# zsyOAOA/VIRNet

Hardware: AMD Instinct MI355X
Metric: images/sec (256x256x3 denoise fwd) (higher is better)
Workload: dtype f32 (3x3 conv products as split-fp16 MFMA pairs, f32 accumulate)

## Files before the change

include/virnet_hip.h:

```cpp
#ifndef VIRNET_HIP_H
#define VIRNET_HIP_H

#include <stddef.h>
#include <stdint.h>

#ifdef __cplusplus
extern "C" {
#endif

#define VIRNET_ABI_VERSION 5

int virnet_abi_version(void);
const char* virnet_last_error(void);
int virnet_device_count(void);

size_t virnet_packed_weight_floats(int ks, int cin_pad, int n_pad);
int virnet_pack_weight(const float* w, int kind, int cout, int cin, int ks, int cin_pad, int n_pad, int nrep,
                       float* packed, void* stream);

typedef struct virnet_conv_plan {
  int nrep;
  int n_pad;
  int cin_pad;
} virnet_conv_plan;
// ... 15 lines not shown
  float* y_raw;
  float* y_act;
  int n, h, w;
  int cin_pad;
  int cout;
  int n_pad;
  int nrep;
  int ks, stride;
  int epi;
  int nchw_op;
  int crop_h, crop_w;
  int res_sf;
  int in_act;
  float in_slope;
  float slope;
  float mask_slope;
  float clamp_lo, clamp_hi;
} virnet_conv_desc;

int virnet_conv_mfma(const virnet_conv_desc* d, void* stream);
int virnet_conv_mfma_variant(const virnet_conv_desc* d, int out[4]);

size_t virnet_wino_weight_floats(int cin_pad, int n_pad);
int virnet_pack_wino_weight(const float* w_oihw, int dgrad, int cout, int cin, int cin_pad, int n_pad, float* packed, void* stream);
int virnet_conv_wino(const virnet_conv_desc* d, void* stream);

size_t virnet_f16_weight_floats(int cin_pad, int n_pad);
int virnet_pack_f16_weight(const float* w_oihw, int dgrad, int cout, int cin, int cin_pad, int n_pad, float* packed, void* stream);
int virnet_conv_f16(const virnet_conv_desc* d, void* stream);
int virnet_pack_bf16_weight(const float* w_oihw, int dgrad, int cout, int cin, int cin_pad, int n_pad, float* packed, void* stream);
int virnet_conv_bf16(const virnet_conv_desc* d, void* stream);
size_t virnet_f16_convt_weight_floats(int cin, int cout);
int virnet_pack_f16_convt_weight(const float* w_iohw, int cout, int cin, float* packed, void* stream);

size_t virnet_wx4_weight_floats(int cin_pad, int n_pad);
int virnet_pack_wx4_weight(const float* w_oihw, int dgrad, int cout, int cin, int cin_pad, int n_pad, float* packed, void* stream);
int virnet_conv_wx4(const virnet_conv_desc* d, void* stream);
void virnet_conv_wx4_last_plan(int* out4);

enum { VIRNET_LAUNCH_WX4 = 0, VIRNET_LAUNCH_WX4H = 1, VIRNET_LAUNCH_WX4P = 2, VIRNET_LAUNCH_F16 = 3, VIRNET_LAUNCH_S2 = 4, VIRNET_LAUNCH_CONVT = 5 };
typedef struct virnet_conv_launch {
  int form, rows, ng, nrep, variant, slab_base, groups, persistent;
} virnet_conv_launch;
enum { VIRNET_PLAN_WX4 = 0, VIRNET_PLAN_F16 = 1, VIRNET_PLAN_BF16 = 2, VIRNET_PLAN_F16_ENTRY = 3 };
int virnet_conv_plan_query(int family, const virnet_conv_desc* d, int emit_rows, int n_cu,
                           virnet_conv_launch* out, int cap);

size_t virnet_exit_weight_floats(int cin_pad);
int virnet_pack_exit_weight(const float* w_oihw, int cout, int cin, int cin_pad, float* packed, void* stream);
int virnet_conv_exit(const virnet_conv_desc* d, void* stream);

int virnet_set_range_flag(int* device_flag);
int virnet_poison_on_flag(const int* device_flag, float* y, size_t n, void* stream);

typedef struct virnet_thin_desc {
  const float* x;
  const float* wpack;
  const float* bias;
  const float* res;
  float* y;
  int n, h, w, c, cout;
  int crop_h, crop_w;
  int op;
  int res_sf;
  float clamp_lo, clamp_hi;
} virnet_thin_desc;
size_t virnet_thin_weight_floats(int c_pad);
int virnet_pack_thin_weight(const float* w_oihw, int cout, int c, int c_pad, float* packed, void* stream);
int virnet_conv3x3_thin(const virnet_thin_desc* d, void* stream);

typedef struct virnet_pack_desc {
  const float* x;
  const float* vec;
  const float* map;
  float* out;
  int n, c0, h, w, sf;
  int ev;
  int em, mh, mw, msf, map_sqrt;
  int hp, wp;
  int zero_pad;
} virnet_pack_desc;
int virnet_pack_input(const virnet_pack_desc* d, void* stream);
int virnet_conv_f16_entry(const virnet_conv_desc* d, const virnet_pack_desc* e, void* stream);
size_t virnet_entry_weight_floats(int cin, int n_pad);
int virnet_pack_entry_weight(const float* w, int cout, int cin, int n_pad, float* packed, void* stream);
int virnet_conv_entry(const virnet_conv_desc* d, const virnet_pack_desc* e, void* stream);

typedef struct virnet_wgrad_desc {
  const float* x;
  const float* dy;
  const float* in_mul;
  const float* in_add;
  float* dw;
  int* counters;
  int n, h, w, cx, cy;
  int cin, cout;
  int ks, stride;
  int transposed;
  int in_act;
  float in_slope;
} virnet_wgrad_desc;
int virnet_conv_wgrad(const virnet_wgrad_desc* d, void* stream);
size_t virnet_chsplit_bytes(int n, int h, int w, int c);
size_t virnet_conv_wgrad_f16_scratch_bytes(int n, int h, int w, int cx, int cy);
size_t virnet_chsplit_colsum_bytes(int n, int h, int w, int c);
int virnet_chsplit(const float* x, int n, int h, int w, int c, int in_act, float in_slope, const float* in_mul, const float* in_add,
// ... 93 lines not shown
```

virnet_amd/_native.py:

```python
from __future__ import annotations

import ctypes as C
import os
import threading

import torch

_HERE = os.path.dirname(os.path.abspath(__file__))
LIB_PATH = os.environ.get("VIRNET_HIP_LIB") or os.path.join(_HERE, "lib", "libvirnet_hip.so")
ABI_VERSION = 5

c_float_p = C.POINTER(C.c_float)


class ConvPlan(C.Structure):
    _fields_ = [("nrep", C.c_int), ("n_pad", C.c_int), ("cin_pad", C.c_int)]


class ConvDesc(C.Structure):
    _fields_ = [
        ("x", C.c_void_p), ("wpack", C.c_void_p), ("bias", C.c_void_p), ("res", C.c_void_p),
        ("mul", C.c_void_p), ("add", C.c_void_p), ("mask", C.c_void_p), ("in_mul", C.c_void_p), ("in_add", C.c_void_p),
        ("y_raw", C.c_void_p), ("y_act", C.c_void_p),
        ("n", C.c_int), ("h", C.c_int), ("w", C.c_int), ("cin_pad", C.c_int), ("cout", C.c_int),
# ... 13 lines not shown

class PackDesc(C.Structure):
    _fields_ = [
        ("x", C.c_void_p), ("vec", C.c_void_p), ("map", C.c_void_p), ("out", C.c_void_p),
        ("n", C.c_int), ("c0", C.c_int), ("h", C.c_int), ("w", C.c_int), ("sf", C.c_int),
        ("ev", C.c_int),
        ("em", C.c_int), ("mh", C.c_int), ("mw", C.c_int), ("msf", C.c_int), ("map_sqrt", C.c_int),
        ("hp", C.c_int), ("wp", C.c_int), ("zero_pad", C.c_int),
    ]


class ImageGradDesc(C.Structure):
    _fields_ = [
        ("dres", C.c_void_p), ("ga", C.c_void_p), ("wa", C.c_void_p), ("gb", C.c_void_p), ("wb", C.c_void_p), ("dx", C.c_void_p),
        ("n", C.c_int), ("c0", C.c_int), ("h", C.c_int), ("w", C.c_int), ("sf", C.c_int),
        ("hp", C.c_int), ("wp", C.c_int), ("ca", C.c_int), ("cina", C.c_int),
        ("cb", C.c_int), ("cinb", C.c_int), ("accumulate", C.c_int),
    ]


class ThinDesc(C.Structure):
    _fields_ = [
        ("x", C.c_void_p), ("wpack", C.c_void_p), ("bias", C.c_void_p), ("res", C.c_void_p), ("y", C.c_void_p),
        ("n", C.c_int), ("h", C.c_int), ("w", C.c_int), ("c", C.c_int), ("cout", C.c_int),
        ("crop_h", C.c_int), ("crop_w", C.c_int), ("op", C.c_int), ("res_sf", C.c_int),
        ("clamp_lo", C.c_float), ("clamp_hi", C.c_float),
    ]


class WgradDesc(C.Structure):
    _fields_ = [
        ("x", C.c_void_p), ("dy", C.c_void_p), ("in_mul", C.c_void_p), ("in_add", C.c_void_p), ("dw", C.c_void_p),
        ("counters", C.c_void_p), ("n", C.c_int), ("h", C.c_int), ("w", C.c_int), ("cx", C.c_int), ("cy", C.c_int),
        ("cin", C.c_int), ("cout", C.c_int), ("ks", C.c_int), ("stride", C.c_int), ("transposed", C.c_int),
        ("in_act", C.c_int), ("in_slope", C.c_float),
    ]


class KnetLayer(C.Structure):
    _fields_ = [(k, C.c_void_p) for k in ("w1pack", "b1", "w2pack", "b2", "caw1", "cab1", "caw2", "cab2")]


class SftWeights(C.Structure):
    _fields_ = [
        ("w1", C.c_void_p), ("b1", C.c_void_p), ("w2", C.c_void_p), ("b2", C.c_void_p),
        ("wm", C.c_void_p), ("bm", C.c_void_p), ("wa", C.c_void_p), ("ba", C.c_void_p),
        ("e", C.c_int), ("nf1", C.c_int), ("nf2", C.c_int), ("nf", C.c_int),
    ]


EPI_NHWC, EPI_CONVT, EPI_NCHW = 0, 1, 2
GAP_MEAN, GAP_EXPCLAMP, GAP_KINFO = 0, 1, 2
NCHW_PLAIN, NCHW_ADD, NCHW_EXPCLAMP = 0, 1, 2
PLAN_WX4, PLAN_F16, PLAN_BF16, PLAN_F16_ENTRY = 0, 1, 2, 3

SYMBOLS = [
    ("virnet_abi_version", C.c_int, []),
    ("virnet_last_error", C.c_char_p, []),
    ("virnet_device_count", C.c_int, []),
    ("virnet_packed_weight_floats", C.c_size_t, [C.c_int, C.c_int, C.c_int]),
    ("virnet_pack_weight", C.c_int, [C.c_void_p, C.c_int, C.c_int, C.c_int, C.c_int, C.c_int, C.c_int, C.c_int,
                                     C.c_void_p, C.c_void_p]),
    ("virnet_conv_get_plan", C.c_int, [C.c_int, C.c_int, C.c_int, C.c_int, C.POINTER(ConvPlan)]),
    ("virnet_conv_mfma", C.c_int, [C.POINTER(ConvDesc), C.c_void_p]),
    ("virnet_conv_mfma_variant", C.c_int, [C.POINTER(ConvDesc), C.POINTER(C.c_int * 4)]),
    ("virnet_wino_weight_floats", C.c_size_t, [C.c_int, C.c_int]),
    ("virnet_pack_wino_weight", C.c_int, [C.c_void_p, C.c_int, C.c_int, C.c_int, C.c_int, C.c_int, C.c_void_p, C.c_void_p]),
    ("virnet_conv_wino", C.c_int, [C.POINTER(ConvDesc), C.c_void_p]),
    ("virnet_f16_weight_floats", C.c_size_t, [C.c_int, C.c_int]),
    ("virnet_pack_f16_weight", C.c_int, [C.c_void_p, C.c_int, C.c_int, C.c_int, C.c_int, C.c_int, C.c_void_p, C.c_void_p]),
    ("virnet_conv_f16", C.c_int, [C.POINTER(ConvDesc), C.c_void_p]),
    ("virnet_wx4_weight_floats", C.c_size_t, [C.c_int, C.c_int]),
    ("virnet_pack_wx4_weight", C.c_int, [C.c_void_p, C.c_int, C.c_int, C.c_int, C.c_int, C.c_int, C.c_void_p, C.c_void_p]),
    ("virnet_conv_wx4", C.c_int, [C.POINTER(ConvDesc), C.c_void_p]),
    ("virnet_conv_wx4_last_plan", None, [C.POINTER(C.c_int)]),
    ("virnet_conv_plan_query", C.c_int, [C.c_int, C.POINTER(ConvDesc), C.c_int, C.c_int, C.POINTER(ConvLaunch), C.c_int]),
    ("virnet_exit_weight_floats", C.c_size_t, [C.c_int]),
    ("virnet_pack_exit_weight", C.c_int, [C.c_void_p, C.c_int, C.c_int, C.c_int, C.c_void_p, C.c_void_p]),
    ("virnet_conv_exit", C.c_int, [C.POINTER(ConvDesc), C.c_void_p]),
    ("virnet_set_range_flag", C.c_int, [C.c_void_p]),
    ("virnet_poison_on_flag", C.c_int, [C.c_void_p, C.c_void_p, C.c_size_t, C.c_void_p]),
    ("virnet_pack_bf16_weight", C.c_int, [C.c_void_p, C.c_int, C.c_int, C.c_int, C.c_int, C.c_int, C.c_void_p, C.c_void_p]),
    ("virnet_conv_bf16", C.c_int, [C.POINTER(ConvDesc), C.c_void_p]),
    ("virnet_f16_convt_weight_floats", C.c_size_t, [C.c_int, C.c_int]),
    ("virnet_pack_f16_convt_weight", C.c_int, [C.c_void_p, C.c_int, C.c_int, C.c_void_p, C.c_void_p]),
    ("virnet_pack_input", C.c_int, [C.POINTER(PackDesc), C.c_void_p]),
    ("virnet_conv_f16_entry", C.c_int, [C.POINTER(ConvDesc), C.POINTER(PackDesc), C.c_void_p]),
    ("virnet_entry_weight_floats", C.c_size_t, [C.c_int, C.c_int]),
    ("virnet_pack_entry_weight", C.c_int, [C.c_void_p, C.c_int, C.c_int, C.c_int, C.c_void_p, C.c_void_p]),
    ("virnet_conv_entry", C.c_int, [C.POINTER(ConvDesc), C.POINTER(PackDesc), C.c_void_p]),
    ("virnet_thin_weight_floats", C.c_size_t, [C.c_int]),
    ("virnet_pack_thin_weight", C.c_int, [C.c_void_p, C.c_int, C.c_int, C.c_int, C.c_void_p, C.c_void_p]),
    ("virnet_conv3x3_thin", C.c_int, [C.POINTER(ThinDesc), C.c_void_p]),
    ("virnet_conv_wgrad", C.c_int, [C.POINTER(WgradDesc), C.c_void_p]),
    ("virnet_sft_backward", C.c_int, [C.c_void_p, C.c_void_p, C.c_void_p, C.c_void_p, C.c_void_p, C.c_float, C.c_void_p, C.c_void_p, C.c_void_p,
                                      C.c_int, C.c_long, C.c_int, C.c_void_p]),
    ("virnet_chsplit_bytes", C.c_size_t, [C.c_int, C.c_int, C.c_int, C.c_int]),
    ("virnet_conv_wgrad_f16_scratch_bytes", C.c_size_t, [C.c_int, C.c_int, C.c_int, C.c_int, C.c_int]),
    ("virnet_chsplit_colsum_bytes", C.c_size_t, [C.c_int, C.c_int, C.c_int, C.c_int]),
    ("virnet_chsplit", C.c_int, [C.c_void_p, C.c_int, C.c_int, C.c_int, C.c_int, C.c_int, C.c_float, C.c_void_p, C.c_void_p, C.c_int,
                                 C.c_void_p, C.c_void_p, C.c_void_p, C.c_int, C.c_void_p]),
    ("virnet_conv_wgrad_f16", C.c_int, [C.c_void_p, C.c_void_p, C.c_void_p, C.c_void_p, C.c_int, C.c_int, C.c_int, C.c_int, C.c_int, C.c_int, C.c_int,
                                        C.c_int, C.c_void_p]),
    ("virnet_chsplit_s2_bytes", C.c_size_t, [C.c_int, C.c_int, C.c_int, C.c_int]),
    ("virnet_chsplit_s2_colsum_bytes", C.c_size_t, [C.c_int, C.c_int, C.c_int, C.c_int]),
    ("virnet_chsplit_s2", C.c_int, [C.c_void_p, C.c_int, C.c_int, C.c_int, C.c_int, C.c_int, C.c_float, C.c_void_p, C.c_void_p, C.c_int,
                                    C.c_void_p, C.c_void_p, C.c_void_p, C.c_int, C.c_void_p]),
    ("virnet_conv_wgrad_f16_s2_scratch_bytes", C.c_size_t, [C.c_int, C.c_int, C.c_int, C.c_int, C.c_int]),
    ("virnet_conv_wgrad_f16_s2", C.c_int, [C.c_void_p, C.c_void_p, C.c_void_p, C.c_void_p, C.c_int, C.c_int, C.c_int, C.c_int, C.c_int, C.c_int,
                                           C.c_int, C.c_int, C.c_int, C.c_void_p]),
    ("virnet_conv_emit_ok", C.c_int, [C.POINTER(ConvDesc), C.c_int, C.POINTER(C.c_int)]),
    ("virnet_conv_f16_emit", C.c_int, [C.POINTER(ConvDesc), C.POINTER(TEmit), C.c_int, C.c_void_p]),
    ("virnet_conv_wx4_emit", C.c_int, [C.POINTER(ConvDesc), C.POINTER(TEmit), C.c_void_p]),
    ("virnet_colpart_reduce", C.c_int, [C.c_void_p, C.c_void_p, C.c_long, C.c_int, C.c_int, C.c_void_p]),
    ("virnet_conv_wgrad_f16_db", C.c_int, [C.c_void_p, C.c_void_p, C.c_void_p, C.c_void_p, C.c_int, C.c_int, C.c_int, C.c_int, C.c_int, C.c_int, C.c_int,
                                           C.c_int, C.c_void_p, C.c_void_p, C.c_long, C.c_int, C.c_void_p]),
    ("virnet_colsum", C.c_int, [C.c_void_p, C.c_void_p, C.c_long, C.c_int, C.c_int, C.c_void_p]),
    ("virnet_zero_stuff2", C.c_int, [C.c_void_p, C.c_void_p, C.c_int, C.c_int, C.c_int, C.c_int, C.c_void_p]),
    ("virnet_space_to_depth2", C.c_int, [C.c_void_p, C.c_void_p, C.c_int, C.c_int, C.c_int, C.c_int, C.c_void_p]),
    ("virnet_pack_input_backward", C.c_int, [C.c_void_p, C.c_int, C.c_int, C.c_void_p, C.c_void_p, C.c_int, C.c_int, C.c_int, C.c_int,
                                             C.c_int, C.c_int, C.c_int, C.c_void_p]),
    ("virnet_image_grad", C.c_int, [C.POINTER(ImageGradDesc), C.c_void_p]),
    ("virnet_conv_head_s4", C.c_int, [C.c_void_p, C.c_void_p, C.c_void_p, C.c_int, C.c_int, C.c_int, C.c_int, C.c_int,
                                      C.c_void_p]),
    ("virnet_conv_head_s4_wgrad", C.c_int, [C.c_void_p, C.c_void_p, C.c_void_p, C.c_int, C.c_int, C.c_int, C.c_int, C.c_int,
                                            C.c_void_p]),
    ("virnet_conv_head_s4_dgrad", C.c_int, [C.c_void_p, C.c_void_p, C.c_void_p, C.c_int, C.c_int, C.c_int, C.c_int, C.c_int,
                                            C.c_void_p]),
    ("virnet_gap_nchw", C.c_int, [C.c_void_p, C.c_void_p, C.c_int, C.c_int, C.c_int, C.c_int, C.c_int, C.c_float,
                                  C.c_float, C.c_void_p]),
    ("virnet_ca_gate", C.c_int, [C.c_void_p, C.c_void_p, C.c_void_p, C.c_void_p, C.c_void_p, C.c_void_p, C.c_int, C.c_int,
                                 C.c_int, C.c_int, C.c_int, C.c_void_p]),
    ("virnet_knet_body", C.c_int, [C.c_void_p, C.c_void_p, C.c_void_p, C.c_int, C.c_int, C.c_int, C.c_int, C.c_int, C.c_int, C.c_void_p]),
    ("virnet_scale_add", C.c_int, [C.c_void_p, C.c_void_p, C.c_void_p, C.c_void_p, C.c_int, C.c_int, C.c_int, C.c_void_p]),
# ... 60 lines not shown
```

virnet_amd/csrc/api.cpp:

```cpp
#include "common.h"
#include <cstdlib>
namespace virnet { int* range_flag_ptr(); int store_nt_for(size_t bytes); }
#include "../../include/virnet_hip.h"

namespace virnet {

char* error_slot() {
  static thread_local char buf[512] = {0};
  return buf;
}

int set_error(const char* fmt, ...) {
  va_list ap;
  va_start(ap, fmt);
  vsnprintf(error_slot(), 512, fmt, ap);
  va_end(ap);
  return 1;
}

static thread_local int* g_range_flag[64] = {nullptr};

int* range_flag_ptr() {
  int dev = 0;
  if (hipGetDevice(&dev) != hipSuccess || dev < 0 || dev > 63) return nullptr;
  return g_range_flag[dev];
}

int store_nt_for(size_t bytes) {
  const char* e = getenv("VIRNET_NT_STORE_MB");
  const long limit = e ? atol(e) : 128;
  return limit > 0 && bytes > (size_t)limit * 1048576u;
}

}

extern "C" int virnet_abi_version(void) { return VIRNET_ABI_VERSION; }

extern "C" const char* virnet_last_error(void) { return virnet::error_slot(); }

extern "C" int virnet_device_count(void) {
  int n = 0;
  hipError_t e = hipGetDeviceCount(&n);
  if (e != hipSuccess) {
    virnet::set_error("hipGetDeviceCount: %s", hipGetErrorString(e));
    return -1;
  }
  return n;
}

extern "C" int virnet_set_range_flag(int* device_flag) {
  int dev = 0;
  hipError_t e = hipGetDevice(&dev);
  if (e != hipSuccess) return virnet::set_error("virnet_set_range_flag: hipGetDevice: %s", hipGetErrorString(e));
  if (dev < 0 || dev > 63) return virnet::set_error("virnet_set_range_flag: device %d out of range", dev);
  virnet::g_range_flag[dev] = device_flag;
  return 0;
}
```

virnet_amd/engine.py:

```python
from __future__ import annotations

from typing import List, Optional, Tuple

import torch

from . import _native as nat
from . import ops

Tensor = torch.Tensor

LOG_MAX = 4.605170185988092
LOG_MIN = -23.025850929940457
K_LOG_MIN = -9.210340371976182


def _prep(x: Tensor, chn: int, name: str = "x") -> Tensor:
    if x.dim() != 4:
        raise ValueError(f"{name} must be [N,C,H,W], got {tuple(x.shape)}")
    if x.shape[1] != chn:
        raise ValueError(f"{name} has {x.shape[1]} channels, the network was built for {chn}")
    if not x.is_cuda:
        raise RuntimeError(f"{name} is on {x.device}: the VIRNet HIP path runs on a ROCm device only (no CPU fallback)")
    if x.dtype != torch.float32:
        raise TypeError(f"{name} must be float32 (the reference is fp32 end to end), got {x.dtype}")
# ... 90 lines not shown
        if ev + em != rnet.extra_chn:
            raise ValueError(f"conditioning has {ev + em} channels, the network was built for {rnet.extra_chn}")
        if extra_map is not None:
            extra_map = _prep(extra_map, em, "extra maps")
        if extra_vec is not None:
            extra_vec = extra_vec.detach().contiguous()
    feed_head = mode in ("input", "both")
    feed_down = mode in ("down", "both")
    cond = None
    rec = None
    if feed_down:
        if extra_map is None:
            cond = _Cond(extra_vec, None, 0, ev)
        else:
            rec = ops.pack_input(x_in, Hp, Wp, sf=sf, vec=extra_vec if feed_head else None,
                                 map_=extra_map if feed_head else None, map_sf=map_sf, map_sqrt=map_sqrt)
            crec = rec if feed_head else ops.pack_input(x_in, Hp, Wp, sf=sf, vec=extra_vec, map_=extra_map,
                                                        map_sf=map_sf, map_sqrt=map_sqrt)
            cond = _Cond(None, crec, rnet.in_chn, ev + em)
    if rec is not None:
        x, _ = ops.conv_mfma(rec, rnet.head.packed(), want_raw=True)
    else:
        x = ops.conv_entry(x_in, rnet.head.packed(), Hp, Wp, sf=sf, vec=extra_vec if feed_head else None,
                           map_=extra_map if feed_head else None, map_sf=map_sf, map_sqrt=map_sqrt)
    if cond is not None and cond.vec is not None and ops._env("VIRNET_SFT_MULTI", "1") != "0":
        atts = [a for lvl in rnet.down_path for blk in lvl.body if blk.extra_chn > 0 for a in (blk.sft1, blk.sft2)]
        if atts:
            cond.pre = {id(a): ma for a, ma in zip(atts, ops.sft_vec_multi(cond.vec, atts))}
    bridges: List[Tensor] = []
    for ii, lvl in enumerate(rnet.down_path):
        for blk in lvl.body:
            x = _res_block(x, blk, cond, ii)
        if ii + 1 < len(rnet.down_path):
            bridges.append(x)
            x, _ = ops.conv_mfma(x, lvl.downsampler.packed(), stride=2, want_raw=True)
    for jj, up in enumerate(rnet.up_path):
        x, _ = ops.conv_mfma(x, up.upsampler.packed(), res=bridges[-jj - 1], want_raw=True)
        for blk in up.body:
            x = _res_block(x, blk, None, 0)
    return _conv_planar(x, rnet.tail, (H, W), op=nat.NCHW_ADD, res=x_in, res_sf=sf)


FP32_FORM = "wino"


class RangeOverflowRepaired(RuntimeWarning):
    """A forward of the deferred guard mode left fp16's range: its outputs were NaN on the device until the repair that this warning
    announces (the same input repeated with the fp32 kernels, written into the same output tensors)."""


_GUARD_WARNING = ("VIRNet HIP path: an activation left fp16's range in a split-fp16 convolution (|x| >= 65504, or >= ~6.5e3 in the "
                  "Winograd form); the forward was repeated with the fp32 kernels")
MAX_PENDING = 2


def guard_check_mode() -> str:
    mode = ops._env("VIRNET_GUARD_CHECK", "sync")
    if mode not in ("sync", "deferred"):
        raise ValueError(f"VIRNET_GUARD_CHECK={mode!r}: expected sync or deferred")
    return mode


def _pending_list() -> list:
    lst = getattr(nat.tls, "guard_pending", None)
    if lst is None:
        lst = nat.tls.guard_pending = []
    return lst


def _settle(block: bool, keep: int = 0) -> None:
    import warnings
    pend = _pending_list()
    while pend:
        pinned, ev, run, outs, dev, stream = pend[0]
        if not ev.query():
            if not block or len(pend) <= keep:
                return
            ev.synchronize()
        pend.pop(0)
        overflowed = bool(int(pinned[0]))
        _pinned_pool().append(pinned)
        if overflowed:
            _GUARD_STATS["reruns"] += 1
            with torch.no_grad(), torch.cuda.device(dev), torch.cuda.stream(stream), ops.forward_scope(form=FP32_FORM):
                res = run()
                for o, r in zip(outs, res if isinstance(res, tuple) else (res,)):
                    o.copy_(r)
            warnings.warn(_GUARD_WARNING + " (deferred check: its outputs were NaN until now)", RangeOverflowRepaired, stacklevel=4)


def _pinned_pool() -> list:
    pool = getattr(nat.tls, "guard_pinned", None)
    if pool is None:
        pool = nat.tls.guard_pinned = []
    return pool


def guard_poll(block: bool = True) -> None:
    _settle(block)


def _range_guarded(run, x: Tensor):
    import warnings
    guarded = ops._f16_family() and ops.range_guard_enabled() and not torch.cuda.is_current_stream_capturing()
    deferred = guarded and guard_check_mode() == "deferred"
    if guarded:
        _settle(block=False)
        flag = ops.range_flag(x.device)
        flag.zero_()
    with ops.forward_scope():
        out = run()
    if deferred:
        outs = out if isinstance(out, tuple) else (out,)
        for o in outs:
            ops.poison_on_flag(flag, o)
        pool = _pinned_pool()
        if pool:
            pinned = pool.pop()
        else:
            with nat.capture_lock:
                pinned = torch.zeros(1, dtype=torch.int32).pin_memory()
        pinned.copy_(flag, non_blocking=True)
        ev = torch.cuda.Event()
        ev.record()
        _pending_list().append((pinned, ev, run, outs, x.device, torch.cuda.current_stream()))
        _settle(block=True, keep=MAX_PENDING)
    elif guarded and ops.range_overflowed(x.device):
        warnings.warn(_GUARD_WARNING, RuntimeWarning, stacklevel=3)
        _GUARD_STATS["reruns"] += 1
        with ops.forward_scope(form=FP32_FORM):
            out = run()
    if guarded:
        _GUARD_STATS["forwards"] += 1
    return out


_GUARD_STATS = {"forwards": 0, "reruns": 0}


def guard_stats(reset: bool = False) -> dict:
    out = dict(_GUARD_STATS)
    if reset:
        _GUARD_STATS["forwards"] = _GUARD_STATS["reruns"] = 0
    return out


def denoise_forward(net, x: Tensor) -> Tuple[Tensor, Tensor]:
    x = _prep(x, net.SNet.in_channels)
    with torch.cuda.device(x.device):
        return _range_guarded(lambda: _denoise_forward(net, x), x)


def _denoise_forward(net, x: Tensor) -> Tuple[Tensor, Tensor]:
    sigma = snet_forward(net.SNet, x, mode="sigma")
    if net.noise_cond:
        if net.SNet.noise_avg:
            raise RuntimeError("VIRAttResUNet(noise_avg=True, noise_cond=True): the [N,C,1,1] variance cannot be "
                               "padded or concatenated with the image (same failure as the reference)")
        mu = rnet_forward(net.RNet, x, extra_map=sigma, map_sqrt=True)
    else:
        mu = rnet_forward(net.RNet, x)
    return mu, sigma


def sisr_forward(net, x: Tensor, sf) -> Tuple[Tensor, Tensor, Tensor]:
    x = _prep(x, net.SNet.in_channels)
    with torch.cuda.device(x.device):
        return _range_guarded(lambda: _sisr_forward(net, x, sf), x)


def _sisr_forward(net, x: Tensor, sf) -> Tuple[Tensor, Tensor, Tensor]:
    if int(sf) != sf or sf < 1:
        raise ValueError(f"sf must be a positive integer, got {sf}")
    sf = int(sf)
    n = x.shape[0]
    sigma = snet_forward(net.SNet, x, mode="sigma")
    kinfo = knet_forward(net.KNet, x)
    vec_parts, emap = [], None
    if net.kernel_cond:
        vec_parts.append(kinfo.view(n, -1))
# ... 9 lines not shown
```

virnet_amd/graph.py:

```python
from __future__ import annotations

import operator
import os
import threading
import warnings
import weakref
from collections import OrderedDict
from typing import Callable, Iterable, Optional, Tuple

import torch

from . import _native as nat
from . import ops


_EPOCH = [0]
FULL_CHECK_EVERY = 64
_VERSIONS = operator.attrgetter("_version")


def _bump(*_a, **_k):
    _EPOCH[0] += 1


def bump_epoch() -> None:
    _EPOCH[0] += 1


_HOOKS = []


def _install_hooks() -> None:
    if not _HOOKS:
        _HOOKS.append(torch.nn.modules.module.register_module_parameter_registration_hook(_bump))
        _HOOKS.append(torch.nn.modules.module.register_module_module_registration_hook(_bump))


_CAPTURE_LOCK = nat.capture_lock


def _env_stamp() -> int:
    data = getattr(os.environ, "_data", None)
    return hash(tuple(data.items())) if data is not None else hash(tuple(sorted(os.environ.items())))


_GRAVEYARD: list = []


def _release(holder=None) -> None:
    with _CAPTURE_LOCK:
        if holder is not None:
            holder.clear()
        del _GRAVEYARD[:]


class RangeOverflow(RuntimeError):
    """Raised by a ``check="deferred"`` GraphedForward when the PREVIOUS replay staged an operand outside fp16's range."""


class GraphedForward:

    def __init__(self, fn: Callable, warmup: int = 2, params: Optional[Callable[[], Iterable[torch.Tensor]]] = None,
                 check: str = "sync", auto_after: int = 0, fresh: bool = False, max_graphs: int = 0):
        if check not in ("sync", "deferred", "off"):
            raise ValueError(f"check={check!r}: expected 'sync', 'deferred' or 'off'")
        _install_hooks()
        self.fn, self.warmup, self.check = fn, warmup, check
        self.auto_after, self.fresh, self.max_graphs = auto_after, fresh, max_graphs
        self._params = params
        self._stamp = None
        self._plist = None
        self._calls = 0
        self._graphs: "OrderedDict[Tuple, Tuple]" = OrderedDict()
        self._seen: dict = {}
        self._pending = None
        self.reruns = 0
        self.replays = 0

    def _walk(self):
        plist = list(self._params())
        return (_EPOCH[0], plist, tuple((id(p), p.data_ptr()) for p in plist))

    def _fingerprint(self):
        if self._params is None:
            return None
        self._calls += 1
        if self._plist is None or self._plist[0] != _EPOCH[0] or self._calls % FULL_CHECK_EVERY == 0:
            self._plist = self._walk()
        return (self._plist[2], tuple(map(_VERSIONS, self._plist[1])))

    def _guard_flag(self, device) -> Optional[torch.Tensor]:
        if self.check == "off" or not (ops._f16_family() and ops.range_guard_enabled()):
            return None
        return ops.range_flag(device)

    def _capture(self, x: torch.Tensor, args: tuple):
        static_x = x.clone()
        flag = self._guard_flag(x.device)
        side = torch.cuda.Stream()
        side.wait_stream(torch.cuda.current_stream())
        with torch.cuda.stream(side), torch.no_grad():
            for _ in range(self.warmup):
                self.fn(static_x, *args)
        torch.cuda.current_stream().wait_stream(side)
        with _CAPTURE_LOCK:
            _sweep_registry()
            _release()
            pinned = torch.zeros(1, dtype=torch.int32).pin_memory() if flag is not None else None
            graph = torch.cuda.CUDAGraph()
            with torch.no_grad(), torch.cuda.graph(graph, capture_error_mode="thread_local"):
                if flag is not None:
                    flag.zero_()
                out = self.fn(static_x, *args)
                out = out if isinstance(out, tuple) else (out,)
                if flag is not None:
                    for o in out:
                        ops.poison_on_flag(flag, o)
                    if pinned is not None and self.check == "sync":
                        pinned.copy_(flag, non_blocking=True)
        return graph, static_x, out, flag, pinned

    def poll(self) -> None:
        if self._pending is None:
            return
        pinned, ev = self._pending
        self._pending = None
        ev.synchronize()
        if int(pinned.item()):
            raise RangeOverflow("the previous graph replay staged an operand outside fp16's range: its outputs are NaN-filled; "
                                "run that input through the eager forward (which repeats it with the fp32 kernels)")

    def __call__(self, x: torch.Tensor, *args):
        if self.check == "deferred":
            self.poll()
        stamp = self._fingerprint()
        if stamp != self._stamp:
            _release(self._graphs)
            self._seen.clear()
            self._stamp = stamp
        key = (tuple(x.shape), x.device.index, args, _env_stamp())
        hit = self._graphs.get(key)
        if hit is None:
            if self.auto_after > 0:
                seen = self._seen.get(key, 0)
                if seen < self.auto_after:
                    if len(self._seen) > 4096:
                        self._seen.clear()
                    self._seen[key] = seen + 1
                    return self.fn(x, *args)
            with torch.cuda.device(x.device):
                hit = self._graphs[key] = self._capture(x, args)
            self._seen.pop(key, None)
            while self.max_graphs > 0 and len(self._graphs) > self.max_graphs:
                with _CAPTURE_LOCK:
                    self._graphs.popitem(last=False)
        elif self.max_graphs > 0:
            self._graphs.move_to_end(key)
        graph, static_x, out, flag, pinned = hit
        static_x.copy_(x)
        graph.replay()
        self.replays += 1
        done = None
        if flag is not None and self.check == "sync":
            done = torch.cuda.Event()
            done.record()
        if self.fresh:
            ret = tuple(torch.empty_like(o) for o in out)
            torch._foreach_copy_(list(ret), list(out))
        else:
            ret = out
        if flag is not None:
            if self.check == "deferred":
                pinned.copy_(flag, non_blocking=True)
                ev = torch.cuda.Event()
                ev.record()
                self._pending = (pinned, ev)
                return ret if len(ret) > 1 else ret[0]
            done.synchronize()
            if int(pinned[0]):
                warnings.warn("VIRNet HIP path: an activation left fp16's range in a replayed graph; this input was repeated eagerly "
                              "with the fp32 kernels", RuntimeWarning, stacklevel=2)
                self.reruns += 1
                from . import engine
                with torch.no_grad(), torch.cuda.device(x.device), ops.forward_scope(form=engine.FP32_FORM):
                    res = self.fn(static_x, *args)
                for o, r in zip(ret, res if isinstance(res, tuple) else (res,)):
                    o.copy_(r)
        return ret if len(ret) > 1 else ret[0]

    def reset(self) -> None:
        _release(self._graphs)
        self._seen.clear()
        self._pending = None

    def __del__(self):
        try:
            _GRAVEYARD.extend(self._graphs.values())
        except Exception:
            pass


AUTO_AFTER = 2


class no_autograph:

    def __enter__(self):
        nat.tls.autograph_off = getattr(nat.tls, "autograph_off", 0) + 1
        return self

    def __exit__(self, *exc):
        nat.tls.autograph_off -= 1
        return False


_REGISTRY: list = []
_REGISTRY_LOCK = threading.Lock()


def _sweep_registry() -> None:
    with _REGISTRY_LOCK:
        dead = [e for e in _REGISTRY if e[0]() is None or not e[1].is_alive()]
        for e in dead:
            _REGISTRY.remove(e)
    for _, _, gf in dead:
        gf.reset()


def _auto_state(module, fn) -> GraphedForward:
    per_thread = getattr(nat.tls, "autograph", None)
    if per_thread is None:
        per_thread = nat.tls.autograph = weakref.WeakKeyDictionary()
# ... 26 lines not shown
```

virnet_amd/ops.py:

```python
from __future__ import annotations

import ctypes as C
import os
from dataclasses import dataclass
from typing import Optional, Tuple

import torch

from . import _native as nat

Tensor = torch.Tensor


@dataclass
class PackedWeight:
    w: Tensor
    bias: Optional[Tensor]
    ks: int
    cout: int
    cin_real: int
    cin_pad: int
    n_pad: int
    nrep: int
    transposed: bool
# ... 133 lines not shown
    if cout < min_cout:
        return False
    th, tw = (h + 15) // 16, (w + 31) // 32
    fill = (h * w) / float(th * 16 * tw * 32)
    if th * tw < min_tiles or fill < min_fill:
        return False
    if deterministic:
        return True
    if n * th * tw * ((cout + 95) // 96) >= min_wgs:
        return True
    return cout % 96 == 0 and n * ((h + 7) // 8) * tw * (cout // 32) >= min_slab_wgs


def pack_wx4_weight(weight: Tensor, *, dgrad: bool = False) -> Tensor:
    lib = nat.load()
    weight = weight.detach()
    _dev_check(weight, "weight")
    cout, cin, kh, kw = weight.shape
    if (kh, kw) != (3, 3):
        raise ValueError("the Winograd form is for 3x3 kernels")
    rows, ks = (cin, cout) if dgrad else (cout, cin)
    if rows % 32:
        raise ValueError(f"virnet_conv_wx4 stores multiples of 32 channels, got {rows}")
    cin_pad = (ks + 15) // 16 * 16
    out = torch.empty(lib.virnet_wx4_weight_floats(cin_pad, rows), dtype=torch.float32, device=weight.device)
    nat.check(lib.virnet_pack_wx4_weight(nat.ptr(weight), int(dgrad), cout, cin, cin_pad, rows, nat.ptr(out), nat.stream_handle()),
              "pack_wx4_weight")
    return out


def wx4_last_plan() -> dict:
    out = (C.c_int * 4)()
    nat.load().virnet_conv_wx4_last_plan(out)
    return {"rows": out[0], "persistent": bool(out[1]), "slabs": out[2], "launches": out[3]}


def conv_plan_query(family: int, desc: "nat.ConvDesc", *, emit_rows: int = 0, n_cu: int = 0) -> list:
    lib = nat.load()
    out = (nat.ConvLaunch * 4)()
    n = lib.virnet_conv_plan_query(family, C.byref(desc), emit_rows, n_cu, out, 4)
    if n < 0:
        nat.check(n, "conv_plan_query")
    return [{k: getattr(out[i], k) for k, _ in nat.ConvLaunch._fields_} for i in range(n)]


def _wino_enabled() -> bool:
    return conv_form() == "wino"


def range_guard_enabled() -> bool:
    return _env("VIRNET_RANGE_GUARD", "1") != "0"


def range_flag(device: torch.device) -> Optional[Tensor]:
    if not range_guard_enabled():
        return None
    idx = device.index if device.index is not None else torch.cuda.current_device()
    flags = getattr(nat.tls, "range_flags", None)
    if flags is None:
        flags = nat.tls.range_flags = {}
    flag = flags.get(idx)
    if flag is None:
        flag = torch.zeros(1, dtype=torch.int32, device=torch.device("cuda", idx))
        with torch.cuda.device(idx):
            nat.check(nat.load().virnet_set_range_flag(nat.ptr(flag)), "set_range_flag")
        flags[idx] = flag
    return flag


def range_overflowed(device: torch.device, *, reset: bool = True) -> bool:
    flag = range_flag(device)
    if flag is None or not bool(flag.item()):
        return False
    if reset:
        flag.zero_()
    return True


def poison_on_flag(flag: Tensor, y: Tensor) -> None:
    nat.check(nat.load().virnet_poison_on_flag(nat.ptr(flag), nat.ptr(y), y.numel(), nat.stream_handle()), "poison_on_flag")


def pack_f16_weight(weight: Tensor, *, dgrad: bool = False, bf16: bool = False) -> Tensor:
    lib = nat.load()
    weight = weight.detach()
    _dev_check(weight, "weight")
    cout, cin, kh, kw = weight.shape
    if (kh, kw) != (3, 3):
        raise ValueError("the split-fp16 form is for 3x3 kernels")
    rows, ks = (cin, cout) if dgrad else (cout, cin)
    n_pad = (rows + 31) // 32 * 32
    cin_pad = (ks + 15) // 16 * 16
    out = torch.empty(lib.virnet_f16_weight_floats(cin_pad, n_pad), dtype=torch.float32, device=weight.device)
    fn = lib.virnet_pack_bf16_weight if bf16 else lib.virnet_pack_f16_weight
    nat.check(fn(nat.ptr(weight), int(dgrad), cout, cin, cin_pad, n_pad, nat.ptr(out), nat.stream_handle()), "pack_f16_weight")
    return out


def pack_wino_weight(weight: Tensor, *, dgrad: bool = False) -> Tensor:
    lib = nat.load()
    weight = weight.detach()
    _dev_check(weight, "weight")
    cout, cin, kh, kw = weight.shape
    if (kh, kw) != (3, 3):
        raise ValueError("the Winograd form is for 3x3 kernels")
    rows, ks = (cin, cout) if dgrad else (cout, cin)
    if rows % 32:
        raise ValueError(f"the Winograd kernel stores multiples of 32 channels, got {rows}")
    cin_pad = (ks + 15) // 16 * 16
    out = torch.empty(lib.virnet_wino_weight_floats(cin_pad, rows), dtype=torch.float32, device=weight.device)
    nat.check(lib.virnet_pack_wino_weight(nat.ptr(weight), int(dgrad), cout, cin, cin_pad, rows, nat.ptr(out), nat.stream_handle()),
              "pack_wino_weight")
    return out


def _dev_check(t: Tensor, name: str) -> None:
    if not t.is_cuda:
        raise RuntimeError(f"{name} is on {t.device}: the VIRNet HIP path needs tensors on a ROCm device "
                           f"(no CPU fallback exists; move the module and inputs with .cuda())")
    if t.dtype != torch.float32:
        raise TypeError(f"{name} must be float32, got {t.dtype}")
    if not t.is_contiguous():
        raise ValueError(f"{name} must be contiguous")


def get_plan(ks: int, stride: int, cin: int, gemm_n: int) -> nat.ConvPlan:
    plan = nat.ConvPlan()
    nat.check(nat.load().virnet_conv_get_plan(ks, stride, cin, gemm_n, C.byref(plan)), "conv_get_plan")
    return plan


def pack_weight(weight: Tensor, bias: Optional[Tensor], *, transposed: bool = False, stride: int = 1,
                dgrad: bool = False) -> PackedWeight:
# ... 875 lines not shown
```

Before: 1590.

## Replace device range flag with mapped pinned host flag slots

The fp16 range-guard flag now lives in host-mapped coherent pinned memory with per-thread slots, so kernels write it directly into host-visible memory. The per-forward device zero_, the pinned copy and the .item() readback are replaced with a host-side store when the stream is idle and a spin on hipStreamQuery followed by an atomic host load. Deferred mode and graphs get dedicated slots with reusable events. This cuts per-forward launches and synchronisation cost, in exchange for kernels doing flag writes over the host-coherent path and added slot-management complexity.

```diff
diff --git a/include/virnet_hip.h b/include/virnet_hip.h
--- a/include/virnet_hip.h
+++ b/include/virnet_hip.h
@@ -91,6 +91,15 @@
 
 int virnet_set_range_flag(int* device_flag);
 int virnet_poison_on_flag(const int* device_flag, float* y, size_t n, void* stream);
+
+#define VIRNET_RANGE_SLOTS 16
+#define VIRNET_RANGE_STRIDE 64
+int virnet_range_select(int slot);
+int* virnet_range_flag_ptr(int slot, int host_side);
+int virnet_range_begin(int slot, void* stream);
+int virnet_range_end(void* stream, int* overflowed);
+int virnet_range_record(void* stream, void** ticket);
+int virnet_range_query(void* ticket, int wait, int* landed, int* overflowed);
 
 typedef struct virnet_thin_desc {
   const float* x;
diff --git a/virnet_amd/_native.py b/virnet_amd/_native.py
--- a/virnet_amd/_native.py
+++ b/virnet_amd/_native.py
@@ -89,6 +89,7 @@
 EPI_NHWC, EPI_CONVT, EPI_NCHW = 0, 1, 2
 GAP_MEAN, GAP_EXPCLAMP, GAP_KINFO = 0, 1, 2
 NCHW_PLAIN, NCHW_ADD, NCHW_EXPCLAMP = 0, 1, 2
+RANGE_SLOTS = 16
 PLAN_WX4, PLAN_F16, PLAN_BF16, PLAN_F16_ENTRY = 0, 1, 2, 3
 
 SYMBOLS = [
@@ -117,6 +118,12 @@
     ("virnet_conv_exit", C.c_int, [C.POINTER(ConvDesc), C.c_void_p]),
     ("virnet_set_range_flag", C.c_int, [C.c_void_p]),
     ("virnet_poison_on_flag", C.c_int, [C.c_void_p, C.c_void_p, C.c_size_t, C.c_void_p]),
+    ("virnet_range_select", C.c_int, [C.c_int]),
+    ("virnet_range_flag_ptr", C.c_void_p, [C.c_int, C.c_int]),
+    ("virnet_range_begin", C.c_int, [C.c_int, C.c_void_p]),
+    ("virnet_range_end", C.c_int, [C.c_void_p, C.POINTER(C.c_int)]),
+    ("virnet_range_record", C.c_int, [C.c_void_p, C.POINTER(C.c_void_p)]),
+    ("virnet_range_query", C.c_int, [C.c_void_p, C.c_int, C.POINTER(C.c_int), C.POINTER(C.c_int)]),
     ("virnet_pack_bf16_weight", C.c_int, [C.c_void_p, C.c_int, C.c_int, C.c_int, C.c_int, C.c_int, C.c_void_p, C.c_void_p]),
     ("virnet_conv_bf16", C.c_int, [C.POINTER(ConvDesc), C.c_void_p]),
     ("virnet_f16_convt_weight_floats", C.c_size_t, [C.c_int, C.c_int]),
diff --git a/virnet_amd/csrc/api.cpp b/virnet_amd/csrc/api.cpp
--- a/virnet_amd/csrc/api.cpp
+++ b/virnet_amd/csrc/api.cpp
@@ -1,5 +1,7 @@
 #include "common.h"
 #include <cstdlib>
+#include <cstring>
+#include <mutex>
 namespace virnet { int* range_flag_ptr(); int store_nt_for(size_t bytes); }
 #include "../../include/virnet_hip.h"
 
@@ -18,12 +20,83 @@
   return 1;
 }
 
-static thread_local int* g_range_flag[64] = {nullptr};
+struct RangeSlot {
+  int* host;
+  int* dev;
+  hipEvent_t ev;
+};
+
+struct RangeBlock {
+  RangeSlot slot[VIRNET_RANGE_SLOTS];
+  RangeBlock* next;
+};
+
+static std::mutex g_range_mutex;
+static RangeBlock* g_range_free[64] = {nullptr};
+
+struct RangeThread {
+  RangeBlock* block[64] = {nullptr};
+  int cur[64] = {0};
+  int* user[64] = {nullptr};
+  bool idle[64] = {false};
+  void* idle_stream[64] = {nullptr};
+  ~RangeThread() {
+    std::lock_guard<std::mutex> lock(g_range_mutex);
+    for (int d = 0; d < 64; ++d)
+      if (block[d]) {
+        block[d]->next = g_range_free[d];
+        g_range_free[d] = block[d];
+      }
+  }
+};
+static thread_local RangeThread g_range;
+
+static int current_device(const char* who, int* dev) {
+  hipError_t e = hipGetDevice(dev);
+  if (e != hipSuccess) return set_error("%s: hipGetDevice: %s", who, hipGetErrorString(e));
+  if (*dev < 0 || *dev > 63) return set_error("%s: device %d out of range", who, *dev);
+  return 0;
+}
+
+static RangeBlock* range_block(int dev) {
+  RangeThread& t = g_range;
+  if (t.block[dev]) return t.block[dev];
+  RangeBlock* b = nullptr;
+  {
+    std::lock_guard<std::mutex> lock(g_range_mutex);
+    b = g_range_free[dev];
+    if (b) g_range_free[dev] = b->next;
+  }
+  if (!b) {
+    void* host = nullptr;
+    void* devp = nullptr;
+    hipError_t e = hipHostMalloc(&host, (size_t)VIRNET_RANGE_SLOTS * VIRNET_RANGE_STRIDE, hipHostMallocMapped | hipHostMallocCoherent);
+    if (e == hipSuccess) e = hipHostGetDevicePointer(&devp, host, 0);
+    if (e != hipSuccess) {
+      set_error("range flag: hipHostMalloc: %s", hipGetErrorString(e));
+      return nullptr;
+    }
+    memset(host, 0, (size_t)VIRNET_RANGE_SLOTS * VIRNET_RANGE_STRIDE);
+    b = new RangeBlock();
+    for (int i = 0; i < VIRNET_RANGE_SLOTS; ++i) {
+      b->slot[i].host = reinterpret_cast<int*>(static_cast<char*>(host) + (size_t)i * VIRNET_RANGE_STRIDE);
+      b->slot[i].dev = reinterpret_cast<int*>(static_cast<char*>(devp) + (size_t)i * VIRNET_RANGE_STRIDE);
+      b->slot[i].ev = nullptr;
+    }
+  }
+  b->next = nullptr;
+  t.block[dev] = b;
+  t.idle[dev] = false;
+  return b;
+}
 
 int* range_flag_ptr() {
   int dev = 0;
   if (hipGetDevice(&dev) != hipSuccess || dev < 0 || dev > 63) return nullptr;
-  return g_range_flag[dev];
+  RangeThread& t = g_range;
+  t.idle[dev] = false;
+  if (t.user[dev]) return t.user[dev];
+  return t.block[dev] ? t.block[dev]->slot[t.cur[dev]].dev : nullptr;
 }
 
 int store_nt_for(size_t bytes) {
@@ -50,9 +123,110 @@
 
 extern "C" int virnet_set_range_flag(int* device_flag) {
   int dev = 0;
-  hipError_t e = hipGetDevice(&dev);
-  if (e != hipSuccess) return virnet::set_error("virnet_set_range_flag: hipGetDevice: %s", hipGetErrorString(e));
-  if (dev < 0 || dev > 63) return virnet::set_error("virnet_set_range_flag: device %d out of range", dev);
-  virnet::g_range_flag[dev] = device_flag;
-  return 0;
-}
+  if (virnet::current_device("virnet_set_range_flag", &dev)) return 1;
+  virnet::g_range.user[dev] = device_flag;
+  virnet::g_range.idle[dev] = false;
+  return 0;
+}
+
+extern "C" int virnet_range_select(int slot) {
+  int dev = 0;
+  if (virnet::current_device("virnet_range_select", &dev)) return 1;
+  VIRNET_REQUIRE(slot >= 0 && slot < VIRNET_RANGE_SLOTS, "virnet_range_select: slot %d out of range", slot);
+  if (!virnet::range_block(dev)) return 1;
+  virnet::g_range.cur[dev] = slot;
+  return 0;
+}
+
+extern "C" int* virnet_range_flag_ptr(int slot, int host_side) {
+  int dev = 0;
+  if (virnet::current_device("virnet_range_flag_ptr", &dev)) return nullptr;
+  if (slot < 0 || slot >= VIRNET_RANGE_SLOTS) {
+    virnet::set_error("virnet_range_flag_ptr: slot %d out of range", slot);
+    return nullptr;
+  }
+  virnet::RangeBlock* b = virnet::range_block(dev);
+  if (!b) return nullptr;
+  return host_side ? b->slot[slot].host : b->slot[slot].dev;
+}
+
+extern "C" int virnet_range_begin(int slot, void* stream) {
+  int dev = 0;
+  if (virnet::current_device("virnet_range_begin", &dev)) return 1;
+  virnet::RangeThread& t = virnet::g_range;
+  hipStream_t s = static_cast<hipStream_t>(stream);
+  if (t.user[dev]) {
+    hipError_t e = hipMemsetAsync(t.user[dev], 0, sizeof(int), s);
+    VIRNET_REQUIRE(e == hipSuccess, "virnet_range_begin: hipMemsetAsync: %s", hipGetErrorString(e));
+    return 0;
+  }
+  if (virnet_range_select(slot)) return 1;
+  const virnet::RangeSlot& w = t.block[dev]->slot[slot];
+  bool host_store = t.idle[dev] && t.idle_stream[dev] == stream;
+  if (host_store) {
+    hipStreamCaptureStatus st = hipStreamCaptureStatusNone;
+    host_store = hipStreamIsCapturing(s, &st) == hipSuccess && st == hipStreamCaptureStatusNone;
+  }
+  if (host_store) {
+    __atomic_store_n(w.host, 0, __ATOMIC_RELEASE);
+  } else {
+    hipError_t e = hipMemsetAsync(w.dev, 0, sizeof(int), s);
+    VIRNET_REQUIRE(e == hipSuccess, "virnet_range_begin: hipMemsetAsync: %s", hipGetErrorString(e));
+  }
+  t.idle[dev] = false;
+  return 0;
+}
+
+extern "C" int virnet_range_end(void* stream, int* overflowed) {
+  int dev = 0;
+  if (virnet::current_device("virnet_range_end", &dev)) return 1;
+  VIRNET_REQUIRE(overflowed != nullptr, "virnet_range_end: NULL pointer");
+  virnet::RangeThread& t = virnet::g_range;
+  VIRNET_REQUIRE(t.user[dev] || t.block[dev], "virnet_range_end: no range flag on device %d in this thread", dev);
+  hipError_t e;
+  while ((e = hipStreamQuery(static_cast<hipStream_t>(stream))) == hipErrorNotReady) __builtin_ia32_pause();
+  VIRNET_REQUIRE(e == hipSuccess, "virnet_range_end: hipStreamQuery: %s", hipGetErrorString(e));
+  if (t.user[dev]) {
+    int v = 0;
+    e = hipMemcpy(&v, t.user[dev], sizeof(int), hipMemcpyDeviceToHost);
+    VIRNET_REQUIRE(e == hipSuccess, "virnet_range_end: hipMemcpy: %s", hipGetErrorString(e));
+    *overflowed = v != 0;
+    return 0;
+  }
+  *overflowed = __atomic_load_n(t.block[dev]->slot[t.cur[dev]].host, __ATOMIC_ACQUIRE) != 0;
+  t.idle[dev] = true;
+  t.idle_stream[dev] = stream;
+  return 0;
+}
+
+extern "C" int virnet_range_record(void* stream, void** ticket) {
+  int dev = 0;
+  if (virnet::current_device("virnet_range_record", &dev)) return 1;
+  VIRNET_REQUIRE(ticket != nullptr, "virnet_range_record: NULL pointer");
+  virnet::RangeThread& t = virnet::g_range;
+  VIRNET_REQUIRE(t.block[dev] && !t.user[dev], "virnet_range_record: the thread's current flag on device %d is not the library's", dev);
+  virnet::RangeSlot& w = t.block[dev]->slot[t.cur[dev]];
+  hipError_t e = hipSuccess;
+  if (!w.ev) e = hipEventCreateWithFlags(&w.ev, hipEventDisableTiming);
+  if (e == hipSuccess) e = hipEventRecord(w.ev, static_cast<hipStream_t>(stream));
+  VIRNET_REQUIRE(e == hipSuccess, "virnet_range_record: %s", hipGetErrorString(e));
+  *ticket = &w;
+  return 0;
+}
+
+extern "C" int virnet_range_query(void* ticket, int wait, int* landed, int* overflowed) {
+  VIRNET_REQUIRE(ticket && landed && overflowed, "virnet_range_query: NULL pointer");
+  virnet::RangeSlot* w = static_cast<virnet::RangeSlot*>(ticket);
+  VIRNET_REQUIRE(w->ev != nullptr, "virnet_range_query: not a recorded ticket");
+  hipError_t e = hipEventQuery(w->ev);
+  if (e == hipErrorNotReady && wait) e = hipEventSynchronize(w->ev);
+  if (e == hipErrorNotReady) {
+    *landed = 0;
+    *overflowed = 0;
+    return 0;
+  }
+  VIRNET_REQUIRE(e == hipSuccess, "virnet_range_query: %s", hipGetErrorString(e));
+  *landed = 1;
+  *overflowed = __atomic_load_n(w->host, __ATOMIC_ACQUIRE) != 0;
+  return 0;
+}
diff --git a/virnet_amd/engine.py b/virnet_amd/engine.py
--- a/virnet_amd/engine.py
+++ b/virnet_amd/engine.py
@@ -166,6 +166,7 @@
 _GUARD_WARNING = ("VIRNet HIP path: an activation left fp16's range in a split-fp16 convolution (|x| >= 65504, or >= ~6.5e3 in the "
                   "Winograd form); the forward was repeated with the fp32 kernels")
 MAX_PENDING = 2
+_DEFERRED_SLOTS = range(1, nat.RANGE_SLOTS)
 
 
 def guard_check_mode() -> str:
@@ -186,14 +187,14 @@
     import warnings
     pend = _pending_list()
     while pend:
-        pinned, ev, run, outs, dev, stream = pend[0]
-        if not ev.query():
+        ticket, slot, run, outs, dev, stream = pend[0]
+        landed, overflowed = ops.range_query(ticket)
+        if not landed:
             if not block or len(pend) <= keep:
                 return
-            ev.synchronize()
+            landed, overflowed = ops.range_query(ticket, wait=True)
         pend.pop(0)
-        overflowed = bool(int(pinned[0]))
-        _pinned_pool().append(pinned)
+        _pinned_pool().append(slot)
         if overflowed:
             _GUARD_STATS["reruns"] += 1
             with torch.no_grad(), torch.cuda.device(dev), torch.cuda.stream(stream), ops.forward_scope(form=FP32_FORM):
@@ -206,7 +207,7 @@
 def _pinned_pool() -> list:
     pool = getattr(nat.tls, "guard_pinned", None)
     if pool is None:
-        pool = nat.tls.guard_pinned = []
+        pool = nat.tls.guard_pinned = list(reversed(_DEFERRED_SLOTS))
     return pool
 
 
@@ -220,26 +221,23 @@
     deferred = guarded and guard_check_mode() == "deferred"
     if guarded:
         _settle(block=False)
-        flag = ops.range_flag(x.device)
-        flag.zero_()
+        slot = 0
+        if deferred:
+            pool = _pinned_pool()
+            while not pool:
+                _settle(block=True, keep=len(_pending_list()) - 1)
+            slot = pool.pop()
+        stream = nat.stream_handle()
+        word = ops.range_begin(x.device, slot, stream)
     with ops.forward_scope():
         out = run()
     if deferred:
         outs = out if isinstance(out, tuple) else (out,)
         for o in outs:
-            ops.poison_on_flag(flag, o)
-        pool = _pinned_pool()
-        if pool:
-            pinned = pool.pop()
-        else:
-            with nat.capture_lock:
-                pinned = torch.zeros(1, dtype=torch.int32).pin_memory()
-        pinned.copy_(flag, non_blocking=True)
-        ev = torch.cuda.Event()
-        ev.record()
-        _pending_list().append((pinned, ev, run, outs, x.device, torch.cuda.current_stream()))
+            ops.poison_on_flag(word, o)
+        _pending_list().append((ops.range_record(stream), slot, run, outs, x.device, torch.cuda.current_stream()))
         _settle(block=True, keep=MAX_PENDING)
-    elif guarded and ops.range_overflowed(x.device):
+    elif guarded and ops.range_end(stream):
         warnings.warn(_GUARD_WARNING, RuntimeWarning, stacklevel=3)
         _GUARD_STATS["reruns"] += 1
         with ops.forward_scope(form=FP32_FORM):
diff --git a/virnet_amd/graph.py b/virnet_amd/graph.py
--- a/virnet_amd/graph.py
+++ b/virnet_amd/graph.py
@@ -74,6 +74,7 @@
         self._graphs: "OrderedDict[Tuple, Tuple]" = OrderedDict()
         self._seen: dict = {}
         self._pending = None
+        self._slot = None
         self.reruns = 0
         self.replays = 0
 
@@ -89,14 +90,24 @@
             self._plist = self._walk()
         return (self._plist[2], tuple(map(_VERSIONS, self._plist[1])))
 
-    def _guard_flag(self, device) -> Optional[torch.Tensor]:
+    def _guard_slot(self) -> Optional[int]:
         if self.check == "off" or not (ops._f16_family() and ops.range_guard_enabled()):
             return None
-        return ops.range_flag(device)
+        if self.check == "sync":
+            return 0
+        if self._slot is None:
+            from . import engine
+            pool = engine._pinned_pool()
+            if len(pool) <= engine.MAX_PENDING + 1:
+                raise RuntimeError("too many check='deferred' GraphedForward objects alive in this thread: no flag word left")
+            self._slot = pool.pop(0)
+            weakref.finalize(self, pool.append, self._slot)
+        return self._slot
 
     def _capture(self, x: torch.Tensor, args: tuple):
         static_x = x.clone()
-        flag = self._guard_flag(x.device)
+        slot = self._guard_slot()
+        flag = None if slot is None else ops.range_word(x.device, slot)
         side = torch.cuda.Stream()
         side.wait_stream(torch.cuda.current_stream())
         with torch.cuda.stream(side), torch.no_grad():
@@ -106,27 +117,24 @@
         with _CAPTURE_LOCK:
             _sweep_registry()
             _release()
-            pinned = torch.zeros(1, dtype=torch.int32).pin_memory() if flag is not None else None
             graph = torch.cuda.CUDAGraph()
             with torch.no_grad(), torch.cuda.graph(graph, capture_error_mode="thread_local"):
                 if flag is not None:
-                    flag.zero_()
+                    ops.range_begin(x.device, slot)
                 out = self.fn(static_x, *args)
                 out = out if isinstance(out, tuple) else (out,)
                 if flag is not None:
                     for o in out:
                         ops.poison_on_flag(flag, o)
-                    if pinned is not None and self.check == "sync":
-                        pinned.copy_(flag, non_blocking=True)
-        return graph, static_x, out, flag, pinned
+        return graph, static_x, out, flag
 
     def poll(self) -> None:
         if self._pending is None:
             return
-        pinned, ev = self._pending
+        flag, ev = self._pending
         self._pending = None
         ev.synchronize()
-        if int(pinned.item()):
+        if flag.host.value:
             raise RangeOverflow("the previous graph replay staged an operand outside fp16's range: its outputs are NaN-filled; "
                                 "run that input through the eager forward (which repeats it with the fp32 kernels)")
 
@@ -156,14 +164,18 @@
                     self._graphs.popitem(last=False)
         elif self.max_graphs > 0:
             self._graphs.move_to_end(key)
-        graph, static_x, out, flag, pinned = hit
+        graph, static_x, out, flag = hit
         static_x.copy_(x)
         graph.replay()
         self.replays += 1
         done = None
-        if flag is not None and self.check == "sync":
+        if flag is not None:
             done = torch.cuda.Event()
-            done.record()
+            if x.device.index == torch.cuda.current_device():
+                done.record()
+            else:
+                with torch.cuda.device(x.device):
+                    done.record()
         if self.fresh:
             ret = tuple(torch.empty_like(o) for o in out)
             torch._foreach_copy_(list(ret), list(out))
@@ -171,13 +183,10 @@
             ret = out
         if flag is not None:
             if self.check == "deferred":
-                pinned.copy_(flag, non_blocking=True)
-                ev = torch.cuda.Event()
-                ev.record()
-                self._pending = (pinned, ev)
+                self._pending = (flag, done)
                 return ret if len(ret) > 1 else ret[0]
             done.synchronize()
-            if int(pinned[0]):
+            if flag.host.value:
                 warnings.warn("VIRNet HIP path: an activation left fp16's range in a replayed graph; this input was repeated eagerly "
                               "with the fp32 kernels", RuntimeWarning, stacklevel=2)
                 self.reruns += 1
diff --git a/virnet_amd/ops.py b/virnet_amd/ops.py
--- a/virnet_amd/ops.py
+++ b/virnet_amd/ops.py
@@ -209,33 +209,78 @@
     return _env("VIRNET_RANGE_GUARD", "1") != "0"
 
 
+class _RangeWord:
+    __slots__ = ("host", "dev")
+
+    def __init__(self, host: int, dev: int):
+        self.host = C.c_int.from_address(host)
+        self.dev = dev
+
+
+def range_word(device: torch.device, slot: int = 0) -> _RangeWord:
+    idx = device.index if device.index is not None else torch.cuda.current_device()
+    words = getattr(nat.tls, "range_words", None)
+    if words is None:
+        words = nat.tls.range_words = {}
+    word = words.get((idx, slot))
+    if word is None:
+        lib = nat.load()
+        with nat.capture_lock, torch.cuda.device(idx):
+            host, dev = lib.virnet_range_flag_ptr(slot, 1), lib.virnet_range_flag_ptr(slot, 0)
+        if not host or not dev:
+            nat.check(1, "range_flag_ptr")
+        word = words[(idx, slot)] = _RangeWord(host, dev)
+    return word
+
+
+def range_begin(device: torch.device, slot: int = 0, stream: Optional[int] = None) -> _RangeWord:
+    word = range_word(device, slot)
+    nat.check(nat.load().virnet_range_begin(slot, nat.stream_handle() if stream is None else stream), "range_begin")
+    return word
+
+
+def range_end(stream: Optional[int] = None) -> bool:
+    out = C.c_int(0)
+    nat.check(nat.load().virnet_range_end(nat.stream_handle() if stream is None else stream, C.byref(out)), "range_end")
+    return bool(out.value)
+
+
+def range_record(stream: Optional[int] = None) -> int:
+    ticket = C.c_void_p(0)
+    nat.check(nat.load().virnet_range_record(nat.stream_handle() if stream is None else stream, C.byref(ticket)), "range_record")
+    return ticket.value
+
+
+def range_query(ticket: int, wait: bool = False) -> Tuple[bool, bool]:
+    landed, over = C.c_int(0), C.c_int(0)
+    nat.check(nat.load().virnet_range_query(ticket, int(wait), C.byref(landed), C.byref(over)), "range_query")
+    return bool(landed.value), bool(over.value)
+
+
 def range_flag(device: torch.device) -> Optional[Tensor]:
     if not range_guard_enabled():
         return None
+    word = range_word(device, 0)
     idx = device.index if device.index is not None else torch.cuda.current_device()
-    flags = getattr(nat.tls, "range_flags", None)
-    if flags is None:
-        flags = nat.tls.range_flags = {}
-    flag = flags.get(idx)
-    if flag is None:
-        flag = torch.zeros(1, dtype=torch.int32, device=torch.device("cuda", idx))
-        with torch.cuda.device(idx):
-            nat.check(nat.load().virnet_set_range_flag(nat.ptr(flag)), "set_range_flag")
-        flags[idx] = flag
-    return flag
+    with torch.cuda.device(idx):
+        nat.check(nat.load().virnet_range_select(0), "range_select")
+    return torch.frombuffer(word.host, dtype=torch.int32)
 
 
 def range_overflowed(device: torch.device, *, reset: bool = True) -> bool:
-    flag = range_flag(device)
-    if flag is None or not bool(flag.item()):
+    if range_flag(device) is None:
         return False
-    if reset:
-        flag.zero_()
-    return True
-
-
-def poison_on_flag(flag: Tensor, y: Tensor) -> None:
-    nat.check(nat.load().virnet_poison_on_flag(nat.ptr(flag), nat.ptr(y), y.numel(), nat.stream_handle()), "poison_on_flag")
+    idx = device.index if device.index is not None else torch.cuda.current_device()
+    with torch.cuda.device(idx):
+        over = range_end()
+    if over and reset:
+        range_word(device, 0).host.value = 0
+    return over
+
+
+def poison_on_flag(flag, y: Tensor) -> None:
+    dev = flag.dev if isinstance(flag, _RangeWord) else nat.ptr(flag)
+    nat.check(nat.load().virnet_poison_on_flag(dev, nat.ptr(y), y.numel(), nat.stream_handle()), "poison_on_flag")
 
 
 def pack_f16_weight(weight: Tensor, *, dgrad: bool = False, bf16: bool = False) -> Tensor:
```

After: 1590, median of 2. About the same (+0.0%).
